# zrc0622/HIRL4UCAV

Hardware: AMD Instinct MI355X
Metric: env steps/sec (whole node) + HIRL update steps/sec at 4096 envs/GPU (higher is better)
Workload: dtype f32

## Files before the change

### hirl4ucav_amd/agents/engine.py

```python
import ctypes
import os

import numpy as np
import torch

from .. import _lib

H1, H2 = 256, 512
_vp, _i32, _f32 = ctypes.c_void_p, ctypes.c_int32, ctypes.c_float


class HxBatch(ctypes.Structure):
    _fields_ = [("rows", _vp), ("bc_rows", _vp), ("batch", _i32), ("noise", _vp)]


class HxSample(ctypes.Structure):
    _fields_ = [("total", _vp), ("cap", ctypes.c_int64), ("ring", _vp), ("expert_ring", _vp), ("expert_len", ctypes.c_int64),
                ("bc_table", _vp), ("bc_len", ctypes.c_int64), ("n_main", _i32), ("seed", ctypes.c_uint64), ("call", ctypes.c_uint32),
                ("sigma", _f32), ("idx", _vp), ("idx_bc", _vp), ("guard", ctypes.c_uint32)]


class HxFront(ctypes.Structure):
    _fields_ = [("flags", _vp), ("status", _vp), ("epoch", ctypes.c_uint32), ("with_c", ctypes.c_uint32)]

# ... 381 lines not shown
        B = self.batch
        if self.needs_reload:
            raise _lib.HxError("this engine failed after a front launch had been enqueued: load a snapshot before learn()")
        st = _lib.stream_ptr()
        pending, self._pending = self._pending, None
        pipe = getattr(before_exchange, "__self__", None) if before_exchange is not None else None
        if pending is not None and pipe is not None and (getattr(pipe, "_armed", None) is not None or getattr(pipe, "issued", False)):
            raise _lib.HxError("sample(defer=True) cannot be combined with an armed VectorStepPipeline: use sample(defer=False) when the "
                               "next env step may run beside learn()")
        if pending is not None and noise is not None:
            raise _lib.HxError("learn(noise=...) after sample(defer=True): the deferred draw produces the smoothing noise itself")
        noise = self._noise if noise is None else noise
        batch = HxBatch(self.rows.data_ptr(), self.bc_rows.data_ptr() if self.use_bc else None, B, noise.data_ptr())
        smp = ctypes.byref(pending[0]) if pending is not None else None
        nets, hyper = ctypes.byref(self.nets), ctypes.byref(self.hyper)
        if bc_weight_now is None:
            w_kind, w_given = 2, 0.0
        elif bc_weight_now == 100:
            w_kind, w_given = 1, 0.0
        else:
            w_kind, w_given = 0, float(bc_weight_now)
        actor_phase = self.actor_trainable
        self.critic_step += 1
        if actor_phase:
            self.actor_step += 1
            self.update_count += 1
        do_polyak = actor_phase and self.update_count % self.target_update_freq == 0
        if not self.staged:
            _lib.call("hx_hirl_learn_sampled", nets, ctypes.byref(batch), hyper, smp, self.critic_step, int(actor_phase), self.actor_step,
                      int(do_polyak), w_kind, w_given, float(bc_warm_up_weight), st)
        else:
            actor_fwd = (2 if w_kind == 1 else 1) if actor_phase else 0
            if smp is not None:
                grads = lambda: _lib.call("hx_hirl_critic_grads_sampled", nets, ctypes.byref(batch), hyper, smp, actor_fwd, st)
            else:
                grads = lambda: _lib.call("hx_hirl_critic_grads", nets, ctypes.byref(batch), hyper, actor_fwd, st)
            self._learn_staged(grads, batch, actor_phase, do_polyak, w_kind, w_given, bc_warm_up_weight, before_exchange)
        self.actor_trainable = not self.actor_trainable

    def _learn_staged(self, critic_grads, batch, actor_phase, do_polyak, w_kind, w_given, bc_warm_up_weight, before_exchange=None):
        B, st = self.batch, _lib.stream_ptr()
        nets, hyper = ctypes.byref(self.nets), ctypes.byref(self.hyper)
        gs = 1.0 / self.world
        own_critic = self.grad_critic.data_ptr()
        if self.xchg is not None:
            self.nets.grad_critic = self.xchg.write_buffer("critic").data_ptr()
        critic_grads()
        if before_exchange is not None:
            before_exchange()
        summed = self._allreduce(self.grad_critic, "critic")
        self.nets.grad_critic = summed.data_ptr()
        pk = 16 if do_polyak else 0
        _lib.call("hx_adam", nets, hyper, 0 | pk, self.critic_step, gs, 0, 0.0, 0.0, B, st)
        self.nets.grad_critic = own_critic
        if actor_phase:
            _lib.call("hx_hirl_actor_backward", nets, ctypes.byref(batch), hyper, int(w_kind == 1), 1, st)
            if self.world > 1 or self.sharded_sequence:
                if self.actor_msg is None:
                    self.actor_msg = torch.zeros(int(_lib.load().hx_actor_message_floats()), dtype=torch.float32, device=self.device)
                msg = self.xchg.write_buffer("actor") if self.xchg is not None else self.actor_msg
                _lib.call("hx_hirl_actor_wgrad_split", nets, hyper, B, msg.data_ptr(), st)
                summed = self._allreduce(msg, "actor")
                _lib.call("hx_adam_mixed", nets, hyper, int(do_polyak), self.actor_step, gs, w_kind, w_given, float(bc_warm_up_weight),
                          B * self.world, summed.data_ptr(), st)
            else:
                _lib.call("hx_hirl_actor_wgrad", nets, hyper, B, B, w_kind, w_given, float(bc_warm_up_weight), st)
                _lib.call("hx_adam", nets, hyper, 1 | pk, self.actor_step, gs, w_kind, w_given, float(bc_warm_up_weight), B, st)

    def step_learn(self, env, expert=None, bc_table=None, n_main=None, act_noise=None, act_sigma=0.0, act_seed=0, out=None, sample_seed=0,
                   smooth_sigma=0.2, bc_weight_now=0.0, bc_warm_up_weight=0.0):
        replay, n, B = env.replay, env.n, self.batch
        bf16 = self.update_dtype == "bf16"
        if replay is None or (self.act_dtype != "bf16" if bf16 else self.act_dtype not in ("f32", "f32x9")):
            raise _lib.HxError("step_learn: the front launch exists for the fp32 networks (acting format 'f32' or 'f32x9') and for the bf16 update path with "
                               "the bf16 acting format, with a replay ring attached to the env")
        if self._pending is not None:
            raise _lib.HxError("step_learn draws its own minibatch: a sample(defer=True) is still pending")
        if self._front is None:
            buf = torch.zeros(96, dtype=torch.int32, device=self.device)
            self._front = (buf[0:64], buf[64:65])
            second = torch.zeros(2 * B * 32 + 2 * B + 64, dtype=torch.float32, device=self.device)
            t2 = (second[:B * 32], second[B * 32:2 * B * 32], second[2 * B * 32:2 * B * 32 + B].view(torch.int32),
                  second[2 * B * 32 + B:2 * B * 32 + 2 * B].view(torch.int32), second[2 * B * 32 + 2 * B:2 * B * 32 + 2 * B + 4])
            self._front_tiles = [(self.rows, self.bc_rows, self._idx, self._idx_bc, self._noise), t2]
        flags, status = self._front
        cur, nxt = self._front_tiles
        n_main = B if n_main is None else int(n_main)
        if self.needs_reload:
            raise _lib.HxError("this engine failed after a front launch had been enqueued (host and device state may disagree): load a snapshot "
                               "(utils/checkpoint.load_run) before stepping it again")
        held = (self._front_epoch, self._front_c_epoch, self.critic_step, self.actor_step, self.update_count, self.sample_calls, self.act_calls, env.steps_issued)
        self._front_enqueued = False
        try:
            return self._step_learn(env, expert, bc_table, n_main, act_noise, act_sigma, act_seed, out, sample_seed, smooth_sigma, bc_weight_now,
                                    bc_warm_up_weight, bf16, flags, status, cur, nxt)
        except _lib.HxError:
            if self._front_enqueued:
                self.needs_reload = True
                raise
            (self._front_epoch, self._front_c_epoch, self.critic_step, self.actor_step, self.update_count, self.sample_calls, self.act_calls, env.steps_issued) = held
            self.front_reset()
            raise

    def _step_learn(self, env, expert, bc_table, n_main, act_noise, act_sigma, act_seed, out, sample_seed, smooth_sigma, bc_weight_now, bc_warm_up_weight,
                    bf16, flags, status, cur, nxt):
        replay, n, B = env.replay, env.n, self.batch
        self.sample_calls += 1

        def draw(tiles, call):
            return HxSample(replay.total.data_ptr(), replay.capacity, replay.ring.data_ptr(), expert.ring.data_ptr() if expert is not None else None,
                            len_of(expert), _lib.ptr(bc_table), bc_table.shape[0] if bc_table is not None else 0, n_main, int(sample_seed), call,
                            float(smooth_sigma), tiles[2].data_ptr(), tiles[3].data_ptr() if bc_table is not None else None, n)

        def tiles_of(t):
            return HxBatch(t[0].data_ptr(), t[1].data_ptr() if self.use_bc else None, B, t[4].data_ptr())

        want = (env, env.steps_issued, replay, expert, bc_table, n_main, int(sample_seed), float(smooth_sigma), self.sample_calls, n)
        if self._front_drawn != want:
            _lib.call("hx_sample_batch_guarded", replay.total.data_ptr(), replay.capacity, replay.ring.data_ptr(), expert.ring.data_ptr() if expert is not None else None,
                      len_of(expert), _lib.ptr(bc_table), bc_table.shape[0] if bc_table is not None else 0, B, n_main, 1, int(sample_seed), self.sample_calls,
                      float(smooth_sigma), cur[2].data_ptr(), cur[3].data_ptr() if bc_table is not None else None, cur[4].data_ptr(), cur[0].data_ptr(),
                      cur[1].data_ptr() if bc_table is not None else None, n, _lib.stream_ptr())
        if out is None:
            out = torch.empty((n, 4), dtype=torch.float32, device=self.device)
        mode = 0
        if act_noise is not None:
            mode = 1 if act_noise.numel() == 4 else 2
        elif act_sigma > 0:
            mode = 3
        self.act_calls += 1
        if self._front_epoch >= 200_000_000:
            flags.zero_()
            self._front_epoch = self._front_c_epoch = 0
        self._front_epoch += 1
        batch, nets, hyper, st = tiles_of(cur), ctypes.byref(self.nets), ctypes.byref(self.hyper), _lib.stream_ptr()
        if bc_weight_now is None:
            w_kind, w_given = 2, 0.0
        elif bc_weight_now == 100:
            w_kind, w_given = 1, 0.0
        else:
            w_kind, w_given = 0, float(bc_weight_now)
        actor_phase = self.actor_trainable
        self.critic_step += 1
        if actor_phase:
            self.actor_step += 1
            self.update_count += 1
        do_polyak = actor_phase and self.update_count % self.target_update_freq == 0
        with_c = int(self.front_c_for(n, actor_phase, w_kind, bf16))
        knob = os.environ.get("HX_FRONT_C")
        carries_c = knob == "1" or (bool(with_c) and knob != "0")
        if carries_c:
            self._front_c_epoch += 1
        front = HxFront(flags.data_ptr(), status.data_ptr(), self._front_epoch, self._front_c_epoch if carries_c else 0)
        _lib.call("hx_hirl_front", env.state.data_ptr(), n, env.pitch, env.obs.data_ptr(), out.data_ptr(), mode | self._mode_bits | (32 if (not bf16 and self._x9_for(n, front=True)) else 0),
                  _lib.ptr(act_noise), float(act_sigma), int(act_seed), int(env.env_id0), self.act_calls, env.reward.data_ptr(), env.done.data_ptr(),
                  env.success.data_ptr(), ctypes.byref(env._opts), nets, ctypes.byref(batch), hyper, int(actor_phase), w_kind, ctypes.byref(front), st)
        self._front_enqueued = True
        env.steps_issued += 1
        nxt_draw, nxt_tiles = draw(nxt, self.sample_calls + 1), tiles_of(nxt)
        if not self.staged:
            _lib.call("hx_hirl_learn_back", nets, ctypes.byref(batch), hyper, self.critic_step, int(actor_phase), self.actor_step, int(do_polyak), w_kind, w_given,
                      float(bc_warm_up_weight), ctypes.byref(nxt_draw), ctypes.byref(nxt_tiles), with_c, st)
        else:
            self._learn_staged(lambda: _lib.call("hx_hirl_critic_grads_back", nets, ctypes.byref(batch), hyper, ctypes.byref(nxt_draw), ctypes.byref(nxt_tiles), with_c, st),
                               batch, actor_phase, do_polyak, w_kind, w_given, bc_warm_up_weight)
        self._front_drawn = (env, env.steps_issued, replay, expert, bc_table, n_main, int(sample_seed), float(smooth_sigma), self.sample_calls + 1, n)
        self._front_tiles = [nxt, cur]
        self.rows, self.bc_rows, self._idx, self._idx_bc, self._noise = cur
        self.actor_trainable = not self.actor_trainable
        return out, env.obs, env.reward, env.done, env.success

    @staticmethod
    def front_waiting_workgroups(batch, with_c=False):
        tiles = (int(batch) + 15) // 16
        return 2 * tiles * 8 + (2 * ((int(batch) + 7) // 8) * 8 if with_c else 0)

    def front_c_for(self, n, actor_phase, w_kind, bf16):
        if self.front_c != "auto":
            return bool(self.front_c)
        if bf16 or not self._x9_for(n, front=True) or n < 8192 or n > 16384:
            return False
        acting = (n + 63) // 64
        jobs = (3 + 2) + (1 + (0 if not self.use_bc else (2 if w_kind == 1 else 1)))
        tiles = (self.batch + 15) // 16
        need = jobs * tiles * 8 * 6.0 + 2 * ((self.batch + 7) // 8) * 8 * 7.6
        return (256 - acting) * 37.0 >= need

    def front_reset(self):
        if self._front is not None:
            self._front[0].zero_()
            self._front[1].zero_()
        self._front_epoch = self._front_c_epoch = 0
        self._front_drawn = None

    def front_status(self):
        return 0 if self._front is None else int(self._front[1].item())

    def front_check(self):
        code = self.front_status()
        if code != 0:
            which = [w for bit, w in ((1, "launch B for the target actor's rows (launch A)"), (2, "launch C for the rows of launches A / B")) if code & bit]
            raise _lib.HxError(f"front launch: an in-launch wait timed out (status word {code}: " + "; ".join(which) + ") - the minibatches read since are "
                               "suspect; the reference-order loop (train_all --loop reference) has no in-launch waits")

    def bc_train_actor(self):
        batch = HxBatch(self.rows.data_ptr(), self.bc_rows.data_ptr(), self.batch, self._noise.data_ptr())
        self.actor_step += 1
        _lib.call("hx_bc_train_actor", ctypes.byref(self.nets), ctypes.byref(batch), ctypes.byref(self.hyper), self.actor_step, _lib.stream_ptr())

    def losses_host(self):
        v = self.losses.tolist()
        return v[0], v[1], v[2], v[3], v[4], v[5]
```

### hirl4ucav_amd/csrc/hx_fwdbwd.hip

```cpp
#include "hx_bwd_body.h"

using namespace hxnn;
using namespace hxu;

namespace {

template <int NT, bool RELU, bool SAMPLE, bool BF16 = false>
__global__ __launch_bounds__(kWide) void fwd_l2_kernel(FwdArgsC A, typename std::conditional<SAMPLE, SampleDev, NoSample>::type SA) {
    __shared__ FwdLds<NT, SAMPLE, BF16> SL;
    fwd_l2_body<NT, RELU, SAMPLE, BF16, 0>(A, SA, (int)blockIdx.x, (int)blockIdx.y, SL, FrontSync{});
}

template <int GRP, bool RELU, bool BF16 = false>
__global__ __launch_bounds__(kWide) void bwd_l2_kernel(BwdArgsC AC) {
    __shared__ BwdLds<GRP, BF16> SL;
    bwd_l2_body<GRP, RELU, BF16, 0>(AC, (int)blockIdx.x, (int)blockIdx.y, SL, FrontSync{});
}


int fwd_row_tiles(const FwdArgs& a) {
    int n = 0;
    for (int j = 0; j < a.njobs; ++j) n += (a.job[j].rows + RT - 1) / RT;
    return n;
}
int bwd_blocks(const BwdArgs& a, int rows_per_wg) {
    return ((a.job[0].rows + rows_per_wg - 1) / rows_per_wg) * kColWgB;
}
template <int GRP>
void launch_bwd_t(const BwdArgs& G, hipStream_t st) {
    BwdArgsC C{};
    for (int j = 0; j < G.njobs; ++j) C.job[j] = pack_bwd(G.job[j], G);
    C.images = G.images;
    static const int rowmap = getenv("HX_XCD_ROWMAP") ? atoi(getenv("HX_XCD_ROWMAP")) : 3;
    C.rowmap = (rowmap >> 1) & 1;
    const dim3 grid(bwd_blocks(G, (GRP <= 2 || GRP >= 4) ? RT / 2 : RT) , G.njobs);
    if constexpr (GRP <= 2) {
        static const int dbg_off = getenv("HX_DBG_BF16_OFF") ? atoi(getenv("HX_DBG_BF16_OFF")) : 0;
        if (G.images && !(dbg_off & 2)) {
            if (G.slope == 0.0f) hipLaunchKernelGGL((bwd_l2_kernel<GRP, true, true>), grid, dim3(kWide), 0, st, C);
            else hipLaunchKernelGGL((bwd_l2_kernel<GRP, false, true>), grid, dim3(kWide), 0, st, C);
            return;
        }
    }
    if (G.slope == 0.0f) hipLaunchKernelGGL((bwd_l2_kernel<GRP, true>), grid, dim3(kWide), 0, st, C);
    else hipLaunchKernelGGL((bwd_l2_kernel<GRP, false>), grid, dim3(kWide), 0, st, C);
}

}

namespace hxu {

static int g_force_fwd_nt = 0, g_force_skip = 0, g_force_count = 0;
void set_fwd_nt(int nt, int skip, int count) { g_force_fwd_nt = nt; g_force_skip = skip; g_force_count = count; }

void launch_fwd(const FwdArgs& F, hipStream_t st) {
    static const bool env64 = getenv("HX_FWD_NT64") && atoi(getenv("HX_FWD_NT64")) != 0;
    bool force64 = env64;
    if (g_force_fwd_nt == kNT) {
        if (g_force_skip > 0) --g_force_skip;
        else if (g_force_count > 0) { --g_force_count; force64 = true; }
    }
    FwdArgsC C{};
    for (int j = 0; j < F.njobs; ++j) {
        C.job[j] = pack_fwd(F.job[j]);
        C.job[j].slope = F.slope;
    }
    C.slope = F.slope; C.zero_nf = F.zero_nf; C.zero_f = F.zero_f; C.zero_i = F.zero_i; C.images = F.images;
    static const int rowmap = getenv("HX_XCD_ROWMAP") ? atoi(getenv("HX_XCD_ROWMAP")) : 3;
    C.rowmap = rowmap & 1;
    const int tiles = fwd_row_tiles(F), per_job = tiles / F.njobs;
    const bool relu = F.slope == 0.0f;
    static const int dbg_off = getenv("HX_DBG_BF16_OFF") ? atoi(getenv("HX_DBG_BF16_OFF")) : 0;
    const bool bf16 = F.images != nullptr && !(dbg_off & 1);
#define HX_FWD_T(NT_, RELU_, BF16_) hipLaunchKernelGGL((fwd_l2_kernel<NT_, RELU_, false, BF16_>), grid, dim3(kWide), 0, st, C, NoSample{})
#define HX_FWD(NT_) do { const dim3 grid(per_job * (H2 / NT_), F.njobs); \
        if (bf16) { if (relu) HX_FWD_T(NT_, true, true); else HX_FWD_T(NT_, false, true); } \
        else { if (relu) HX_FWD_T(NT_, true, false); else HX_FWD_T(NT_, false, false); } } while (0)
    if (F.sample) {
        const dim3 grid(per_job * (H2 / kNT), F.njobs);
        if (bf16) {
            if (relu) hipLaunchKernelGGL((fwd_l2_kernel<kNT, true, true, true>), grid, dim3(kWide), 0, st, C, *F.sample);
            else hipLaunchKernelGGL((fwd_l2_kernel<kNT, false, true, true>), grid, dim3(kWide), 0, st, C, *F.sample);
        } else {
            if (relu) hipLaunchKernelGGL((fwd_l2_kernel<kNT, true, true>), grid, dim3(kWide), 0, st, C, *F.sample);
            else hipLaunchKernelGGL((fwd_l2_kernel<kNT, false, true>), grid, dim3(kWide), 0, st, C, *F.sample);
        }
        return;
    }
    if (tiles >= 128) HX_FWD(256);
    else if (tiles * (H2 / 32) <= 256 && !force64) HX_FWD(32);
    else HX_FWD(kNT);
#undef HX_FWD_T
#undef HX_FWD
}

void launch_bwd(int grp, const BwdArgs& G, hipStream_t st) {
    switch (grp) {
        case 0: launch_bwd_t<0>(G, st); break;
        case 1: launch_bwd_t<1>(G, st); break;
        case 2: launch_bwd_t<2>(G, st); break;
        case 4: launch_bwd_t<4>(G, st); break;
        case 5: launch_bwd_t<5>(G, st); break;
        default: launch_bwd_t<3>(G, st); break;
    }
}

}

HX_DEFINE_DEBUG_COLLECTORS(fwdbwd, 0, 32)

extern "C" int hx_debug_set_fwd_nt(int32_t nt, int32_t skip, int32_t count) {
    HX_REQUIRE((nt == 0 || nt == 64) && skip >= 0 && count >= 0, "hx_debug_set_fwd_nt: nt 0 or 64, skip and count >= 0");
    hxu::set_fwd_nt(nt, skip, count);
    return 0;
}
```

### hirl4ucav_amd/csrc/hx_hirl.hip

```cpp
#include <cmath>

#include "hx_update.h"

using namespace hxnn;
using namespace hxu;

extern "C" {

int hx_actor_param_count(void) { return kActor.size(); }
int hx_critic_param_count(void) { return 2 * kQ.padded(); }
int64_t hx_hirl_workspace_floats(int32_t batch) { return (int64_t)S_COUNT * kSlotFloats * batch + 64; }
int64_t hx_actor_message_floats(void) { return 2 * (int64_t)kActor.padded() + 64; }
int64_t hx_bf16_images_elems(void) { return (int64_t)IM_COUNT * (int64_t)kImgElems; }

int hx_pack_update_images(const HxNets* N, void* stream) {
    HX_REQUIRE(N && N->w2_bf16_all && (reinterpret_cast<uintptr_t>(N->w2_bf16_all) & 15u) == 0, "hx_pack_update_images: w2_bf16_all must be a 16-byte aligned buffer");
    HX_REQUIRE(N->actor && N->critic && N->target_actor && N->target_critic, "hx_pack_update_images: null network");
    hipStream_t st = (hipStream_t)stream;
    uint16_t* im = N->w2_bf16_all;
    launch_pack_bf16(N->actor + kActor.W2(), im + IM_ACTOR * kImgElems, false, st);
    launch_pack_bf16(N->actor + kActor.W2(), im + IM_ACTOR_T * kImgElems, true, st);
    launch_pack_bf16(N->target_actor + kActor.W2(), im + IM_TA * kImgElems, false, st);
    if (N->bc_actor) launch_pack_bf16(N->bc_actor + kActor.W2(), im + IM_BC * kImgElems, false, st);
    for (int h = 0; h < 2; ++h) {
        launch_pack_bf16(N->critic + h * kQ.padded() + kQ.W2(), im + (IM_C1 + h) * kImgElems, false, st);
        launch_pack_bf16(N->critic + h * kQ.padded() + kQ.W2(), im + (IM_C1_T + h) * kImgElems, true, st);
        launch_pack_bf16(N->target_critic + h * kQ.padded() + kQ.W2(), im + (IM_TC1 + h) * kImgElems, false, st);
    }
    HX_CHECK_LAUNCH("hx_pack_update_images");
    return 0;
}

static void make_slots(const HxNets* N, int B, Slot* s) {
    for (int i = 0; i < S_COUNT; ++i) s[i] = carve_slot(N->ws + (size_t)i * kSlotFloats * B, B);
}

static WgAdam make_adam(const HxNets* N, const HxHyper* Hy, float lr, int step, bool finish_actor) {
    const double b1 = 0.9, b2 = 0.999;
    const double bc1 = 1.0 - pow(b1, step), bc2 = 1.0 - pow(b2, step);
    WgAdam a{};
    a.b1 = (float)b1; a.b2 = (float)b2; a.eps = 1e-8f;
    a.step_size = (float)(lr / bc1);
    a.bc2_sqrt = (float)sqrt(bc2);
    a.tau = Hy->tau;
    a.finish_actor = finish_actor ? 1 : 0;
    a.use_bc = Hy->use_bc;
    a.losses = N->losses;
    a.wstate = N->wstate;
    return a;
}

static void make_launch_a(const HxNets* N, const HxBatch* Bt, const HxHyper* Hy, int32_t actor_fwd, FwdArgs& F) {
    const Mlp mA{13, 4, Hy->no_layernorm ? 1 : 0}, mQ{17, 1, Hy->no_layernorm ? 1 : 0};
    const int B = Bt->batch;
    Slot s[S_COUNT];
    make_slots(N, B, s);
    const RowSrc src{Bt->rows, nullptr, nullptr, 0, 32};
    F = FwdArgs{};
    F.njobs = 3; F.slope = Hy->slope;
    F.zero_f = N->losses; F.zero_nf = 1;
    F.job[0] = FwdJob{N->target_actor, mA, src, 17, 0, Head{}, nullptr, 0.f, s[S_TA], B, 0, IM_TA};
    F.job[1] = FwdJob{N->critic, mQ, src, 0, 0, Head{}, nullptr, 0.f, s[S_C1], B, 1, IM_C1};
    F.job[2] = FwdJob{N->critic + mQ.padded(), mQ, src, 0, 0, Head{}, nullptr, 0.f, s[S_C2], B, 1, IM_C2};
    if (actor_fwd) {
        F.zero_nf = 5; F.zero_i = N->soft_count;
        F.job[3] = FwdJob{N->actor, mA, src, 0, 0, Head{}, nullptr, 0.f, s[S_API], B, 1, IM_ACTOR};
        F.njobs = 4;
    }
    F.images = N->w2_bf16_all;
}
static void make_launch_b(const HxNets* N, const HxBatch* Bt, const HxHyper* Hy, int32_t actor_fwd, FwdArgs& F) {
    const Mlp mA{13, 4, Hy->no_layernorm ? 1 : 0}, mQ{17, 1, Hy->no_layernorm ? 1 : 0};
    const int B = Bt->batch;
    Slot s[S_COUNT];
    make_slots(N, B, s);
    const RowSrc src{Bt->rows, nullptr, nullptr, 0, 32};
    const float* tc1 = N->target_critic;
    const float* tc2 = N->target_critic + mQ.padded();
    F = FwdArgs{};
    F.njobs = 2; F.slope = Hy->slope;
    const Head prev{N->target_actor, mA, s[S_TA]};
    F.job[0] = FwdJob{tc1, mQ, src, 17, 1, prev, Bt->noise, Hy->noise_clamp, s[S_TC1], B, 0, IM_TC1};
    F.job[1] = FwdJob{tc2, mQ, src, 17, 1, prev, Bt->noise, Hy->noise_clamp, s[S_TC2], B, 0, IM_TC2};
    if (actor_fwd && Hy->use_bc) {
        const RowSrc bcsrc{Bt->bc_rows ? Bt->bc_rows : Bt->rows, nullptr, nullptr, 0, 32};
        int n = 2;
        F.job[n++] = FwdJob{N->actor, mA, bcsrc, 0, 0, Head{}, nullptr, 0.f, s[S_ABC], B, 1, IM_ACTOR};
        if (actor_fwd == 2) F.job[n++] = FwdJob{N->bc_actor, mA, src, 0, 0, Head{}, nullptr, 0.f, s[S_BCS], B, 0, IM_BC};
        F.njobs = n;
    }
    F.images = N->w2_bf16_all;
}
static void make_launch_c(const HxNets* N, const HxBatch* Bt, const HxHyper* Hy, BwdArgs& G) {
    const Mlp mQ{17, 1, Hy->no_layernorm ? 1 : 0};
    const int B = Bt->batch;
    Slot s[S_COUNT];
    make_slots(N, B, s);
    const RowSrc src{Bt->rows, nullptr, nullptr, 0, 32};
    const float* tc1 = N->target_critic;
    const float* tc2 = N->target_critic + mQ.padded();
    G = BwdArgs{};
    G.njobs = 2; G.slope = Hy->slope; G.inv_batch = 1.0f / B; G.losses = N->losses; G.soft_count = N->soft_count;
    for (int h = 0; h < 2; ++h) {
        BwdJob& J = G.job[h];
        J = BwdJob{};
        J.net = N->critic + h * mQ.padded(); J.m = mQ; J.ws = s[S_C1 + h]; J.rows = B; J.mode = BM_CRITIC_TD;
        J.t1 = Head{tc1, mQ, s[S_TC1]}; J.t2 = Head{tc2, mQ, s[S_TC2]}; J.src = src; J.gamma = Hy->gamma;
        J.img_t = IM_C1_T + h;
    }
    G.images = N->w2_bf16_all;
}
static bool front_has_c(bool asked) {
    static const int force = getenv("HX_FRONT_C") ? atoi(getenv("HX_FRONT_C")) : -1;
    return force < 0 ? asked : force != 0;
}
static int critic_back(const HxNets* N, const HxBatch* Bt, const HxHyper* Hy, void* stream, int adam_step, bool polyak, const SampleDev* predraw = nullptr, bool skip_c = false) {
    hipStream_t st = (hipStream_t)stream;
    const Mlp mQ{17, 1, Hy->no_layernorm ? 1 : 0};
    const int B = Bt->batch;
    Slot s[S_COUNT];
    make_slots(N, B, s);
    if (!skip_c) {
        BwdArgs G;
        make_launch_c(N, Bt, Hy, G);
        launch_bwd(0, G, st);
    }
    {
        WgArgs W{};
        W.njobs = 2; W.slope = Hy->slope; W.w_kind = 0; W.w_given = 0.f; W.inv_batch = 1.0f / B;
        W.soft_count = N->soft_count; W.wstate = N->wstate;
        for (int h = 0; h < 2; ++h) {
            WgJob& J = W.job[h];
            J = WgJob{};
            J.net = N->critic + h * mQ.padded(); J.grad = N->grad_critic + h * mQ.padded(); J.m = mQ;
            J.ws[0] = s[S_C1 + h]; J.rows[0] = B; J.nslots = 1; J.wmode[0] = 0;
            if (adam_step > 0) {
                J.p = N->critic + h * mQ.padded();
                J.mom = N->m_critic + h * mQ.padded(); J.var = N->v_critic + h * mQ.padded();
                J.target = polyak ? N->target_critic + h * mQ.padded() : nullptr;
                if (uint16_t* im = N->w2_bf16_all) {
                    J.w2b = im + (IM_C1 + h) * kImgElems; J.w2tb = im + (IM_C1_T + h) * kImgElems; J.tgt_w2b = im + (IM_TC1 + h) * kImgElems;
                }
            }
        }
        W.bf16 = N->w2_bf16_all != nullptr;
        W.predraw = predraw; W.predraw_batch = B;
        if (adam_step > 0) {
            W.ad = make_adam(N, Hy, Hy->lr_critic, adam_step, false);
            launch_wg(W, true, st);
        } else {
            launch_wg(W, false, st);
        }
    }
    HX_CHECK_LAUNCH("hx_hirl_critic_grads");
    return 0;
}
static int critic_grads_impl(const HxNets* N, const HxBatch* Bt, const HxHyper* Hy, int32_t actor_fwd, void* stream, int adam_step, bool polyak,
                             const HxSample* S = nullptr) {
    HX_REQUIRE(N && Bt && Hy && Bt->batch > 0 && Bt->batch % 16 == 0, "hx_hirl_critic_grads: batch must be a positive multiple of 16");
    hipStream_t st = (hipStream_t)stream;
    const int B = Bt->batch;
    SampleDev SD{};
    bool fused = false;
    if (S) {
        HX_REQUIRE(Bt->noise, "hx_hirl_*_sampled: the draw needs the output word noise[4]");
        if (int rc = prepare_draw(S, B, const_cast<float*>(Bt->rows), const_cast<float*>(Bt->bc_rows), const_cast<float*>(Bt->noise), stream, &SD, &fused)) return rc;
    }
    FwdArgs F;
    make_launch_a(N, Bt, Hy, actor_fwd, F);
    F.sample = fused ? &SD : nullptr;
    launch_fwd(F, st);
    make_launch_b(N, Bt, Hy, actor_fwd, F);
    launch_fwd(F, st);
    return critic_back(N, Bt, Hy, stream, adam_step, polyak);
}
int hx_hirl_critic_grads(const HxNets* N, const HxBatch* Bt, const HxHyper* Hy, int32_t actor_fwd, void* stream) {
    return critic_grads_impl(N, Bt, Hy, actor_fwd, stream, 0, false);
}
int hx_hirl_critic_grads_sampled(const HxNets* N, const HxBatch* Bt, const HxHyper* Hy, const HxSample* S, int32_t actor_fwd, void* stream) {
    HX_REQUIRE(S, "hx_hirl_critic_grads_sampled: null sample description");
    return critic_grads_impl(N, Bt, Hy, actor_fwd, stream, 0, false, S);
}

int hx_hirl_actor_backward(const HxNets* N, const HxBatch* Bt, const HxHyper* Hy, int32_t estimate_soft, int32_t fwd_done, void* stream) {
    HX_REQUIRE(N && Bt && Hy && Bt->batch > 0 && Bt->batch % 16 == 0, "hx_hirl_actor_backward: batch must be a positive multiple of 16");
    hipStream_t st = (hipStream_t)stream;
    const Mlp mA{13, 4, Hy->no_layernorm ? 1 : 0}, mQ{17, 1, Hy->no_layernorm ? 1 : 0};
    (void)mA; (void)mQ;
    const int B = Bt->batch;
    Slot s[S_COUNT];
    make_slots(N, B, s);
    const RowSrc src{Bt->rows, nullptr, nullptr, 0, 32};
    const RowSrc bcsrc{Bt->bc_rows ? Bt->bc_rows : Bt->rows, nullptr, nullptr, 0, 32};
    const bool bc = Hy->use_bc != 0, soft = bc && estimate_soft;
    if (!fwd_done) {
        FwdArgs F{};
        F.slope = Hy->slope;
        F.zero_f = N->losses + 1; F.zero_nf = 4; F.zero_i = N->soft_count;
        int n = 0;
        F.job[n++] = FwdJob{N->actor, mA, src, 0, 0, Head{}, nullptr, 0.f, s[S_API], B, 1, IM_ACTOR};
        if (bc) F.job[n++] = FwdJob{N->actor, mA, bcsrc, 0, 0, Head{}, nullptr, 0.f, s[S_ABC], B, 1, IM_ACTOR};
        if (soft) F.job[n++] = FwdJob{N->bc_actor, mA, src, 0, 0, Head{}, nullptr, 0.f, s[S_BCS], B, 0, IM_BC};
        F.njobs = n;
        F.images = N->w2_bf16_all;
        launch_fwd(F, st);
    }
    {
        FwdArgs F{};
        F.slope = Hy->slope;
        int n = 0;
        F.job[n++] = FwdJob{N->critic, mQ, src, 0, 1, Head{N->actor, mA, s[S_API]}, nullptr, 0.f, s[S_CPI], B, 1, IM_C1};
        if (soft) F.job[n++] = FwdJob{N->critic, mQ, src, 0, 1, Head{N->bc_actor, mA, s[S_BCS]}, nullptr, 0.f, s[S_CSOFT], B, 0, IM_C1};
        F.njobs = n;
        F.images = N->w2_bf16_all;
        launch_fwd(F, st);
    }
    {
        BwdArgs G{};
        G.njobs = 1; G.slope = Hy->slope; G.inv_batch = 1.0f / B; G.losses = N->losses; G.soft_count = N->soft_count;
        BwdJob& J = G.job[0];
        J = BwdJob{};
        J.net = N->critic; J.m = mQ; J.ws = s[S_CPI]; J.rows = B; J.mode = BM_CRITIC_PI;
        if (soft) J.soft = Head{N->critic, mQ, s[S_CSOFT]};
        J.img_t = IM_C1_T;
        G.images = N->w2_bf16_all;
        launch_bwd(1, G, st);
    }
    {
        BwdArgs G{};
        G.slope = Hy->slope; G.inv_batch = 1.0f / B; G.losses = N->losses; G.soft_count = N->soft_count;
        int n = 0;
        {
            BwdJob& J = G.job[n++];
            J = BwdJob{};
            J.net = N->actor; J.m = mA; J.ws = s[S_API]; J.rows = B; J.mode = BM_ACTOR_PI;
            J.crit = Head{N->critic, mQ, s[S_CPI]};
            J.img_t = IM_ACTOR_T;
        }
        if (bc) {
            BwdJob& J = G.job[n++];
            J = BwdJob{};
            J.net = N->actor; J.m = mA; J.ws = s[S_ABC]; J.rows = B; J.mode = BM_ACTOR_BC;
            J.src = bcsrc; J.lambda = Hy->loss_lambda;
            J.img_t = IM_ACTOR_T;
        }
        G.njobs = n;
        G.images = N->w2_bf16_all;
        launch_bwd(2, G, st);
    }
    HX_CHECK_LAUNCH("hx_hirl_actor_backward");
    return 0;
}

static int actor_wgrad_impl(const HxNets* N, const HxHyper* Hy, int32_t batch, int32_t count_batch, int32_t w_kind, float w_given,
                            float warm, void* stream, int adam_step, bool polyak) {
    HX_REQUIRE(N && Hy && batch > 0 && count_batch > 0, "hx_hirl_actor_wgrad: bad arguments");
    const Mlp mA{13, 4, Hy->no_layernorm ? 1 : 0}, mQ{17, 1, Hy->no_layernorm ? 1 : 0};
    (void)mA; (void)mQ;
    Slot s[S_COUNT];
    make_slots(N, batch, s);
    const bool bc = Hy->use_bc != 0;
    WgArgs W{};
    W.njobs = 1; W.slope = Hy->slope; W.w_kind = bc ? w_kind : 0; W.w_given = bc ? w_given : 0.0f; W.warm = warm;
    W.inv_batch = 1.0f / count_batch; W.soft_count = N->soft_count; W.wstate = N->wstate;
    WgJob& J = W.job[0];
    J = WgJob{};
    J.net = N->actor; J.grad = N->grad_actor; J.m = mA;
    J.ws[0] = s[S_API]; J.rows[0] = batch; J.wmode[0] = 1;
    J.nslots = 1;
    if (bc) { J.ws[1] = s[S_ABC]; J.rows[1] = batch; J.wmode[1] = 2; J.nslots = 2; }
    W.bf16 = N->w2_bf16_all != nullptr;
    if (adam_step > 0) {
        J.p = N->actor; J.mom = N->m_actor; J.var = N->v_actor;
        J.target = polyak ? N->target_actor : nullptr;
        J.w2b = N->actor_w2_bf16;
        J.w2f = N->actor_w2_f32i;
        if (N->actor_w2_x9) {
            HX_REQUIRE(!N->actor_w2_bf16 && !N->w2_bf16_all, "hx_hirl_learn: actor_w2_x9 excludes the plain bf16 images (one acting format at a time)");
            J.w2b = N->actor_w2_x9; J.w2b_x9 = 1;
        }
        if (uint16_t* im = N->w2_bf16_all) {
            HX_REQUIRE(!N->actor_w2_bf16 || N->actor_w2_bf16 == im + IM_ACTOR * kImgElems, "hx_hirl_learn: with w2_bf16_all set, actor_w2_bf16 must be NULL or its first image");
            J.w2b = im + IM_ACTOR * kImgElems; J.w2tb = im + IM_ACTOR_T * kImgElems; J.tgt_w2b = im + IM_TA * kImgElems;
        }
        W.ad = make_adam(N, Hy, Hy->lr_actor, adam_step, true);
        launch_wg(W, true, (hipStream_t)stream);
    } else {
        launch_wg(W, false, (hipStream_t)stream);
    }
    HX_CHECK_LAUNCH("hx_hirl_actor_wgrad");
    return 0;
}
int hx_hirl_actor_wgrad(const HxNets* N, const HxHyper* Hy, int32_t batch, int32_t count_batch, int32_t w_kind, float w_given,
                        float warm, void* stream) {
    return actor_wgrad_impl(N, Hy, batch, count_batch, w_kind, w_given, warm, stream, 0, false);
}

int hx_hirl_actor_wgrad_split(const HxNets* N, const HxHyper* Hy, int32_t batch, float* msg, void* stream) {
    HX_REQUIRE(N && Hy && batch > 0 && msg && (reinterpret_cast<uintptr_t>(msg) & 15u) == 0, "hx_hirl_actor_wgrad_split: bad arguments");
    const Mlp mA{13, 4, Hy->no_layernorm ? 1 : 0}, mQ{17, 1, Hy->no_layernorm ? 1 : 0};
    (void)mA; (void)mQ;
    Slot s[S_COUNT];
    make_slots(N, batch, s);
    const bool bc = Hy->use_bc != 0;
    WgArgs W{};
    W.njobs = bc ? 2 : 1; W.slope = Hy->slope; W.w_kind = 0; W.w_given = 0.0f; W.inv_batch = 1.0f / batch;
    W.soft_count = N->soft_count; W.wstate = N->wstate;
    for (int j = 0; j < W.njobs; ++j) {
        WgJob& J = W.job[j];
        J = WgJob{};
        J.net = N->actor; J.grad = msg + j * mA.padded(); J.m = mA;
        J.ws[0] = s[j == 0 ? S_API : S_ABC]; J.rows[0] = batch; J.wmode[0] = 0; J.nslots = 1;
    }
    W.bf16 = N->w2_bf16_all != nullptr;
    W.soft_count = bc ? N->soft_count : nullptr;
    W.count_out = msg + 2 * mA.padded();
    launch_wg(W, false, (hipStream_t)stream);
    HX_CHECK_LAUNCH("hx_hirl_actor_wgrad_split");
    return 0;
}

int hx_hirl_learn(const HxNets* N, const HxBatch* Bt, const HxHyper* Hy, int32_t critic_step, int32_t actor_phase,
                  int32_t actor_step, int32_t do_polyak, int32_t w_kind, float w_given, float warm, void* stream) {
    return hx_hirl_learn_sampled(N, Bt, Hy, nullptr, critic_step, actor_phase, actor_step, do_polyak, w_kind, w_given, warm, stream);
}
int hx_hirl_learn_sampled(const HxNets* N, const HxBatch* Bt, const HxHyper* Hy, const HxSample* S, int32_t critic_step, int32_t actor_phase,
                          int32_t actor_step, int32_t do_polyak, int32_t w_kind, float w_given, float warm, void* stream) {
    HX_REQUIRE(critic_step >= 1 && (!actor_phase || actor_step >= 1), "hx_hirl_learn: Adam steps are 1-based");
    int rc = critic_grads_impl(N, Bt, Hy, actor_phase ? (w_kind == 1 ? 2 : 1) : 0, stream, critic_step, do_polyak != 0, S);
    if (rc || !actor_phase) return rc;
    if ((rc = hx_hirl_actor_backward(N, Bt, Hy, w_kind == 1, 1, stream))) return rc;
    return actor_wgrad_impl(N, Hy, Bt->batch, Bt->batch, w_kind, w_given, warm, stream, actor_step, do_polyak != 0);
}

int hx_hirl_front(float* state, int64_t n, int64_t stride, float* obs_io, float* actions, int32_t noise_mode, const float* noise,
                  float sigma, uint64_t seed, uint32_t row0, uint32_t call, float* reward, uint8_t* done, int8_t* success, const HxStepOpts* opts,
                  const HxNets* N, const HxBatch* Bt, const HxHyper* Hy, int32_t actor_phase, int32_t w_kind, const HxFront* front, void* stream) {
    HX_REQUIRE(N && Bt && Hy && front && opts && Bt->batch > 0 && Bt->batch % 16 == 0 && Bt->batch <= kFusedBatchMax && Bt->rows && Bt->noise,
               "hx_hirl_front: the minibatch tiles (a positive multiple of 16 rows, at most 256) and noise[4] must be there");
    HX_REQUIRE(front->flags && front->status && front->epoch >= 1, "hx_hirl_front: flags, status and a 1-based epoch are required");
    const bool bf16 = N->w2_bf16_all != nullptr;
    HX_REQUIRE(bf16 ? N->actor_w2_bf16 != nullptr : (!N->actor_w2_bf16 && (N->actor_w2_f32i || N->actor_w2_x9)),
               "hx_hirl_front: fp32 networks with HxNets.actor_w2_f32i / actor_w2_x9, or the bf16 update path (w2_bf16_all) with actor_w2_bf16");
    const int actor_fwd = actor_phase ? (w_kind == 1 ? 2 : 1) : 0;
    FwdArgs FA, FB;
    make_launch_a(N, Bt, Hy, actor_fwd, FA);
    make_launch_b(N, Bt, Hy, actor_fwd, FB);
    const bool x9 = !bf16 && (noise_mode & 32) != 0;
    HX_REQUIRE(bf16 || (x9 ? N->actor_w2_x9 != nullptr : N->actor_w2_f32i != nullptr), "hx_hirl_front: the image of the chosen acting format is missing from HxNets");
    noise_mode &= ~32;
    BwdArgs GC;
    const bool with_c = front_has_c(front->with_c != 0);
    HX_REQUIRE(!with_c || front->with_c != 0, "hx_hirl_front: HX_FRONT_C=1 needs a caller that counts its launches with launch C (HxFront.with_c = 1, 2, ...)");
    if (with_c) make_launch_c(N, Bt, Hy, GC);
    return launch_front(N->actor, (x9 || bf16) ? nullptr : N->actor_w2_f32i, x9 ? N->actor_w2_x9 : nullptr, bf16 ? N->actor_w2_bf16 : nullptr, state, n, stride, obs_io, actions, noise_mode, noise, sigma, seed,
                        row0, call, Hy->slope, reward, done, success, *opts, FA, FB, with_c ? &GC : nullptr, *front, (hipStream_t)stream);
}
static int make_predraw(const HxNets* N, const HxBatch* Bt, const HxSample* next, const HxBatch* next_tiles, void* stream, SampleDev* SD) {
    HX_REQUIRE(next_tiles && next_tiles->batch == Bt->batch && next_tiles->rows && next_tiles->noise && next_tiles->rows != Bt->rows && next_tiles->noise != Bt->noise,
               "hx_hirl_learn_back: the next minibatch needs tiles of its own (this call still reads the current ones)");
    (void)N;
    bool fused = false;
    if (int rc = prepare_draw(next, Bt->batch, const_cast<float*>(next_tiles->rows), const_cast<float*>(next_tiles->bc_rows), const_cast<float*>(next_tiles->noise),
                              stream, SD, &fused, false)) return rc;
    HX_REQUIRE(fused, "hx_hirl_learn_back: the predraw covers minibatches of at most 256 rows");
    return 0;
}
int hx_hirl_critic_grads_back(const HxNets* N, const HxBatch* Bt, const HxHyper* Hy, const HxSample* next, const HxBatch* next_tiles, int32_t c_in_front,
                              void* stream) {
    HX_REQUIRE(N && Bt && Hy && Bt->batch > 0 && Bt->batch % 16 == 0, "hx_hirl_critic_grads_back: batch must be a positive multiple of 16");
    SampleDev SD{};
    if (next) if (int rc = make_predraw(N, Bt, next, next_tiles, stream, &SD)) return rc;
    return critic_back(N, Bt, Hy, stream, 0, false, next ? &SD : nullptr, front_has_c(c_in_front != 0));
}
int hx_hirl_learn_back(const HxNets* N, const HxBatch* Bt, const HxHyper* Hy, int32_t critic_step, int32_t actor_phase, int32_t actor_step, int32_t do_polyak,
                       int32_t w_kind, float w_given, float warm, const HxSample* next, const HxBatch* next_tiles, int32_t c_in_front, void* stream) {
    HX_REQUIRE(N && Bt && Hy && Bt->batch > 0 && Bt->batch % 16 == 0, "hx_hirl_learn_back: batch must be a positive multiple of 16");
    HX_REQUIRE(critic_step >= 1 && (!actor_phase || actor_step >= 1), "hx_hirl_learn_back: Adam steps are 1-based");
    SampleDev SD{};
    if (next) if (int rc = make_predraw(N, Bt, next, next_tiles, stream, &SD)) return rc;
    int rc = critic_back(N, Bt, Hy, stream, critic_step, do_polyak != 0, next ? &SD : nullptr, front_has_c(c_in_front != 0));
    if (rc || !actor_phase) return rc;
    if ((rc = hx_hirl_actor_backward(N, Bt, Hy, w_kind == 1, 1, stream))) return rc;
    return actor_wgrad_impl(N, Hy, Bt->batch, Bt->batch, w_kind, w_given, warm, stream, actor_step, do_polyak != 0);
}

int hx_bc_train_actor(const HxNets* N, const HxBatch* Bt, const HxHyper* Hy, int32_t step, void* stream) {
    HX_REQUIRE(N && Bt && Hy && Bt->bc_rows && Bt->batch > 0 && Bt->batch % 16 == 0 && step >= 1, "hx_bc_train_actor: bad arguments");
    hipStream_t st = (hipStream_t)stream;
    const Mlp mA{13, 4, Hy->no_layernorm ? 1 : 0}, mQ{17, 1, Hy->no_layernorm ? 1 : 0};
    (void)mA; (void)mQ;
    const int B = Bt->batch;
    Slot s[S_COUNT];
    make_slots(N, B, s);
    const RowSrc bcsrc{Bt->bc_rows, nullptr, nullptr, 0, 32};
    {
        FwdArgs F{};
        F.njobs = 1; F.slope = Hy->slope;
        F.zero_f = N->losses + 1; F.zero_nf = 4;
        F.job[0] = FwdJob{N->actor, mA, bcsrc, 0, 0, Head{}, nullptr, 0.f, s[S_ABC], B, 1, IM_ACTOR};
        F.images = N->w2_bf16_all;
        launch_fwd(F, st);
    }
    {
        BwdArgs G{};
        G.njobs = 1; G.slope = Hy->slope; G.inv_batch = 1.0f / B; G.losses = N->losses; G.soft_count = N->soft_count;
        BwdJob& J = G.job[0];
        J = BwdJob{};
        J.net = N->actor; J.m = mA; J.ws = s[S_ABC]; J.rows = B; J.mode = BM_ACTOR_BC; J.src = bcsrc; J.lambda = 1.0f;
        J.img_t = IM_ACTOR_T;
        G.images = N->w2_bf16_all;
        launch_bwd(2, G, st);
    }
    {
        WgArgs W{};
        W.njobs = 1; W.slope = Hy->slope; W.w_kind = 0; W.w_given = 0.f; W.inv_batch = 1.0f / B;
        W.soft_count = N->soft_count; W.wstate = N->wstate;
        WgJob& J = W.job[0];
        J = WgJob{};
        J.net = N->actor; J.grad = N->grad_actor; J.m = mA; J.ws[0] = s[S_ABC]; J.rows[0] = B; J.nslots = 1; J.wmode[0] = 0;
        W.bf16 = N->w2_bf16_all != nullptr;
        launch_wg(W, false, st);
    }
    HX_CHECK_LAUNCH("hx_bc_train_actor");
    return hx_adam(N, Hy, 2, step, 1.0f, 0, 0.0f, 0.0f, B, stream);
}

}
```

### hirl4ucav_amd/csrc/hx_update.h

```cpp
#pragma once
#include <cstdlib>
#include <type_traits>

#include "hx_common.h"
#include "hx_nn.h"

#ifdef HX_STAMPS
static __device__ float hx_dbg[80];
#define STAMP_DECL unsigned long long TS_[16]; int tsn_ = 0
#define STAMP() TS_[tsn_++] = __builtin_amdgcn_s_memrealtime()
#define STAMP_FLUSH(base, cond) do { if (cond) { for (int i_ = 1; i_ < tsn_; ++i_) hx_dbg[(base) + i_] = (float)(TS_[i_] - TS_[i_ - 1]); hx_dbg[(base)] = (float)tsn_; } } while (0)
constexpr int kSpanCap = 8192;
static __device__ unsigned long long hx_span[kSpanCap][2];
static __device__ unsigned hx_span_tag[kSpanCap];
static __device__ unsigned hx_span_n;
#define SPAN_LOG(tag) do { if (threadIdx.x == 0) { const unsigned long long e_ = __builtin_amdgcn_s_memrealtime(); const unsigned i_ = atomicAdd(&hx_span_n, 1u); \
    if (i_ < (unsigned)kSpanCap) { hx_span[i_][0] = TS_[0]; hx_span[i_][1] = e_; hx_span_tag[i_] = (unsigned)(tag) | (blockIdx.x << 8) | (blockIdx.y << 24); } } } while (0)
#define HX_DEFINE_DEBUG_COLLECTORS(name, lo, hi) \
    namespace hx { \
    int dbg_stamps_##name(float* host80) { \
        float tmp[80]; \
        if (hipMemcpyFromSymbol(tmp, HIP_SYMBOL(hx_dbg), sizeof(tmp)) != hipSuccess) return -2; \
        for (int i = (lo); i < (hi); ++i) host80[i] = tmp[i]; \
        return 0; \
// ... 428 lines not shown
#pragma clang fp contract(off)
__device__ __forceinline__ void sac_policy_dout(float da, float a, float se, float mask, float ab, float& d_mean, float& d_logstd) {
    const float t = 1.0f - a * a;
    const float dHdx = (-2.0f * a * t) / (t + 1e-6f);
    const float dLdx = da * t - ab * dHdx;
    d_mean = dLdx;
    d_logstd = (dLdx * se - ab) * mask;
}
#pragma clang fp contract(fast)

struct BwdJob {
    const float* net;
    Mlp m;
    Slot ws;
    int rows;
    int mode;
    Head t1, t2;
    RowSrc src;
    float gamma;
    Head soft;
    Head crit;
    float lambda;
    const float* bonus;
    const float* bonus_scale;
    int loss_slot;
    int img_t;
};
struct BwdArgs {
    BwdJob job[2];
    int njobs;
    float slope;
    float inv_batch;
    float* losses;
    int* soft_count;
    const uint16_t* images;
};

struct WgJob {
    const float* net;
    float* grad;
    Mlp m;
    Slot ws[2];
    int rows[2];
    int nslots;
    int wmode[2];
    float* p; float* mom; float* var;
    float* target;
    uint16_t* w2b;
    float* w2f;
    uint16_t* w2tb;
    uint16_t* tgt_w2b;
    int w2b_x9;
};
struct WgAdam {
    float b1, b2, eps, step_size, bc2_sqrt, tau;
    int finish_actor, use_bc;
    float* losses;
    float* wstate;
    float* alpha_state;
    float target_entropy, alpha_step_size;
};
struct WgArgs {
    WgJob job[2];
    int njobs;
    float slope;
    WgAdam ad;
    int w_kind;
    float w_given, warm, inv_batch;
    const int* soft_count;
    const float* wstate;
    int bf16;
    float* count_out;
    const SampleDev* predraw;
    int predraw_batch;
};

#pragma clang fp contract(off)
__device__ __forceinline__ void adam_update(float& p, float& m, float& v, float g, float b1, float b2, float eps, float step_size, float bc2_sqrt) {
    m = __builtin_fmaf(g, 1.0f - b1, m * b1);
    v = __builtin_fmaf(g * g, 1.0f - b2, v * b2);
    const float denom = __builtin_amdgcn_sqrtf(v) * __builtin_amdgcn_rcpf(bc2_sqrt) + eps;
    p = p - step_size * (m * __builtin_amdgcn_rcpf(denom));
}
__device__ __forceinline__ float polyak_update(float target, float p, float tau) { return target * (1.0f - tau) + p * tau; }
#pragma clang fp contract(fast)
__device__ __forceinline__ float effective_w(int kind, float given, float warm, float inv_batch, const int* count, const float* wstate) {
    float w = given;
    if (kind == 1) w = (float)(*count) * inv_batch + warm;
    if (kind == 2) w = *wstate;
    return w > 1.0f ? 1.0f : w;
}

struct AdamArgs {
    float* p; const float* g; float* m; float* v;
    int n;
    float b1, b2, eps, step_size, bc2_sqrt, gscale;
    int finish_actor;
    int w_kind; float w_given, warm, inv_batch;
    const int* soft_count; float* wstate; float* losses; int use_bc;
    float* alpha_state;
    float target_entropy, alpha_step_size;
    float* target;
    float tau;
    uint16_t* w2b;
    float* w2f;
    int w2b_x9;
    int w2_lo;
    int nseg;
    int seg_lo[2];
    uint16_t* seg_w2b[2];
    uint16_t* seg_w2tb[2];
    uint16_t* seg_tgt_w2b[2];
    const float* g2;
    const float* countf;
    const uint32_t* guard;
};

constexpr size_t kSlotFloats = XP + H1 + 2 + H1 + H2 + 2 + OW + H2 + H1 + OW + 2 * kColWgB;

enum { S_TA = 0, S_C1, S_C2, S_TC1, S_TC2, S_API, S_ABC, S_BCS, S_CPI, S_CSOFT, S_COUNT };

const Mlp kActor{13, 4, 0};
const Mlp kQ{17, 1, 0};
const Mlp kPolicy{13, 8, 1};
const Mlp kQs{17, 1, 1};

__device__ __forceinline__ float pick8(const float (&o)[8], int i) {
    return i == 0 ? o[0] : i == 1 ? o[1] : i == 2 ? o[2] : i == 3 ? o[3] : i == 4 ? o[4] : i == 5 ? o[5] : i == 6 ? o[6] : o[7];
}

inline int prepare_draw(const HxSample* S, int B, float* rows, float* bc_rows, float* noise, void* stream, SampleDev* SD, bool* fused, bool launch_now = true) {
    HX_REQUIRE(S->total && S->cap > 0 && S->ring && S->idx && rows && S->n_main >= 0 && S->n_main <= B,
               "hx_*_sampled: the draw needs total, cap, ring, idx and the output tile rows");
    HX_REQUIRE(S->n_main == B || S->expert_ring, "hx_*_sampled: expert rows requested without an expert ring");
    HX_REQUIRE(!S->bc_table == !S->idx_bc && (!S->bc_table || bc_rows), "hx_*_sampled: bc_table, idx_bc and bc_rows go together");
    *fused = B <= kFusedBatchMax;
    HX_REQUIRE(!S->guard || *fused, "hx_*_sampled: HxSample.guard is honoured by the fused draw only (batch <= 256)");
    HX_REQUIRE(!S->guard || 2 * (int64_t)S->guard <= S->cap, "hx_*_sampled: a guard of more than half the ring leaves too little to draw from (cap >= 2 n)");
    if (*fused) {
        *SD = SampleDev{(const unsigned long long*)S->total, S->ring, S->expert_ring ? S->expert_ring : S->ring, S->bc_table, rows,
                        S->bc_table ? bc_rows : nullptr, noise, S->idx, S->idx_bc, (long long)S->cap, (uint32_t)S->expert_len, (uint32_t)S->bc_len,
                        S->n_main, S->call, S->seed, S->sigma, S->guard};
        return 0;
    }
    if (!launch_now) return 0;
    return hx_sample_batch(S->total, S->cap, S->ring, S->expert_ring, S->expert_len, S->bc_table, S->bc_len, B, S->n_main, 1, S->seed, S->call,
                           S->sigma, S->idx, S->idx_bc, noise, rows, S->bc_table ? bc_rows : nullptr, stream);
}


void launch_fwd(const FwdArgs& F, hipStream_t st);
void set_fwd_nt(int nt, int skip, int count);
void launch_bwd(int grp, const BwdArgs& G, hipStream_t st);
int launch_front(const float* actor, const float* w2f, const uint16_t* w2x, const uint16_t* w2b, float* state, int64_t n, int64_t stride, float* obs_io, float* actions, int32_t noise_mode,
                 const float* noise, float sigma, uint64_t seed, uint32_t row0, uint32_t call, float slope, float* reward, uint8_t* done, int8_t* success,
                 const HxStepOpts& o, const FwdArgs& FA, const FwdArgs& FB, const BwdArgs* GC, const HxFront& front, hipStream_t st);
void launch_wg(const WgArgs& W, bool adam, hipStream_t st);
void launch_adam(const AdamArgs& A, hipStream_t st);
void launch_polyak(float* target, const float* source, int n, float tau, float* target2, const float* source2, int n2, hipStream_t st,
                   const uint32_t* guard = nullptr);
void launch_pack_bf16(const float* w2, uint16_t* image, bool transposed, hipStream_t st);

}
```

Before: 79.59 million.

## Move BC actor forward from front launch B into actor backward launch H

In the non-staged actor phase with behaviour cloning enabled, the BC-rows actor forward job is removed from the front's launch B. It is instead co-launched with the first actor backward layer-2 kernel in one grid, where some blocks run the backward and the rest run the forward, sharing LDS through a union. This shortens the front's forward launch and fills the backward launch with independent work. The risk is a larger LDS footprint and uneven block mix in the combined kernel, plus the BC forward output now being ready later than before.

After: 79.67 million (median of 6 runs). No clear change (+0.1%).

```diff
diff --git a/hirl4ucav_amd/agents/engine.py b/hirl4ucav_amd/agents/engine.py
--- a/hirl4ucav_amd/agents/engine.py
+++ b/hirl4ucav_amd/agents/engine.py
@@ -557,7 +557,8 @@
         if carries_c:
             self._front_c_epoch += 1
         front = HxFront(flags.data_ptr(), status.data_ptr(), self._front_epoch, self._front_c_epoch if carries_c else 0)
-        _lib.call("hx_hirl_front", env.state.data_ptr(), n, env.pitch, env.obs.data_ptr(), out.data_ptr(), mode | self._mode_bits | (32 if (not bf16 and self._x9_for(n, front=True)) else 0),
+        sbc_in_h = not self.staged and actor_phase and self.use_bc
+        _lib.call("hx_hirl_front", env.state.data_ptr(), n, env.pitch, env.obs.data_ptr(), out.data_ptr(), mode | self._mode_bits | (32 if (not bf16 and self._x9_for(n, front=True)) else 0) | (64 if sbc_in_h else 0),
                   _lib.ptr(act_noise), float(act_sigma), int(act_seed), int(env.env_id0), self.act_calls, env.reward.data_ptr(), env.done.data_ptr(),
                   env.success.data_ptr(), ctypes.byref(env._opts), nets, ctypes.byref(batch), hyper, int(actor_phase), w_kind, ctypes.byref(front), st)
         self._front_enqueued = True
@@ -565,7 +566,7 @@
         nxt_draw, nxt_tiles = draw(nxt, self.sample_calls + 1), tiles_of(nxt)
         if not self.staged:
             _lib.call("hx_hirl_learn_back", nets, ctypes.byref(batch), hyper, self.critic_step, int(actor_phase), self.actor_step, int(do_polyak), w_kind, w_given,
-                      float(bc_warm_up_weight), ctypes.byref(nxt_draw), ctypes.byref(nxt_tiles), with_c, st)
+                      float(bc_warm_up_weight), ctypes.byref(nxt_draw), ctypes.byref(nxt_tiles), with_c | (2 if sbc_in_h else 0), st)
         else:
             self._learn_staged(lambda: _lib.call("hx_hirl_critic_grads_back", nets, ctypes.byref(batch), hyper, ctypes.byref(nxt_draw), ctypes.byref(nxt_tiles), with_c, st),
                                batch, actor_phase, do_polyak, w_kind, w_given, bc_warm_up_weight)
diff --git a/hirl4ucav_amd/csrc/hx_fwdbwd.hip b/hirl4ucav_amd/csrc/hx_fwdbwd.hip
--- a/hirl4ucav_amd/csrc/hx_fwdbwd.hip
+++ b/hirl4ucav_amd/csrc/hx_fwdbwd.hip
@@ -15,6 +15,20 @@
 __global__ __launch_bounds__(kWide) void bwd_l2_kernel(BwdArgsC AC) {
     __shared__ BwdLds<GRP, BF16> SL;
     bwd_l2_body<GRP, RELU, BF16, 0>(AC, (int)blockIdx.x, (int)blockIdx.y, SL, FrontSync{});
+}
+
+template <bool RELU, bool BF16>
+__global__ __launch_bounds__(kWide) void bwd1_fwd_kernel(BwdArgsC AC, int nb, FwdArgsC F) {
+    __shared__ union {
+        BwdLds<1, BF16> b;
+        FwdLds<kNT, false, BF16> f;
+    } u;
+    const int b = (int)blockIdx.x;
+    if (b < nb) {
+        bwd_l2_body<1, RELU, BF16, 0>(AC, b, 0, u.b, FrontSync{});
+        return;
+    }
+    fwd_l2_body<kNT, RELU, false, BF16, 0>(F, NoSample{}, b - nb, 0, u.f, FrontSync{});
 }
 
 
@@ -94,6 +108,30 @@
 #undef HX_FWD
 }
 
+int launch_bwd1_fwd(const BwdArgs& G, const FwdArgs& F, hipStream_t st) {
+    HX_REQUIRE(G.njobs == 1 && F.njobs == 1 && !F.sample && F.zero_nf == 0 && !F.zero_i && F.job[0].rows == G.job[0].rows && !G.images == !F.images,
+               "launch_bwd1_fwd: one backward job of launch H and one forward job on the same minibatch, the same update path");
+    BwdArgsC C{};
+    C.job[0] = pack_bwd(G.job[0], G);
+    C.images = G.images;
+    static const int rowmap = getenv("HX_XCD_ROWMAP") ? atoi(getenv("HX_XCD_ROWMAP")) : 3;
+    C.rowmap = (rowmap >> 1) & 1;
+    FwdArgsC A{};
+    A.job[0] = pack_fwd(F.job[0]);
+    A.job[0].slope = F.slope;
+    A.slope = F.slope; A.images = F.images; A.rowmap = rowmap & 1;
+    const int nb = bwd_blocks(G, RT / 2), nf = ((F.job[0].rows + RT - 1) / RT) * (H2 / kNT);
+    const dim3 grid((unsigned)(nb + nf));
+    if (G.images) {
+        if (G.slope == 0.0f) hipLaunchKernelGGL((bwd1_fwd_kernel<true, true>), grid, dim3(kWide), 0, st, C, nb, A);
+        else hipLaunchKernelGGL((bwd1_fwd_kernel<false, true>), grid, dim3(kWide), 0, st, C, nb, A);
+    } else {
+        if (G.slope == 0.0f) hipLaunchKernelGGL((bwd1_fwd_kernel<true, false>), grid, dim3(kWide), 0, st, C, nb, A);
+        else hipLaunchKernelGGL((bwd1_fwd_kernel<false, false>), grid, dim3(kWide), 0, st, C, nb, A);
+    }
+    return 0;
+}
+
 void launch_bwd(int grp, const BwdArgs& G, hipStream_t st) {
     switch (grp) {
         case 0: launch_bwd_t<0>(G, st); break;
diff --git a/hirl4ucav_amd/csrc/hx_hirl.hip b/hirl4ucav_amd/csrc/hx_hirl.hip
--- a/hirl4ucav_amd/csrc/hx_hirl.hip
+++ b/hirl4ucav_amd/csrc/hx_hirl.hip
@@ -69,7 +69,7 @@
     }
     F.images = N->w2_bf16_all;
 }
-static void make_launch_b(const HxNets* N, const HxBatch* Bt, const HxHyper* Hy, int32_t actor_fwd, FwdArgs& F) {
+static void make_launch_b(const HxNets* N, const HxBatch* Bt, const HxHyper* Hy, int32_t actor_fwd, FwdArgs& F, bool sbc_in_h = false) {
     const Mlp mA{13, 4, Hy->no_layernorm ? 1 : 0}, mQ{17, 1, Hy->no_layernorm ? 1 : 0};
     const int B = Bt->batch;
     Slot s[S_COUNT];
@@ -85,7 +85,7 @@
     if (actor_fwd && Hy->use_bc) {
         const RowSrc bcsrc{Bt->bc_rows ? Bt->bc_rows : Bt->rows, nullptr, nullptr, 0, 32};
         int n = 2;
-        F.job[n++] = FwdJob{N->actor, mA, bcsrc, 0, 0, Head{}, nullptr, 0.f, s[S_ABC], B, 1, IM_ACTOR};
+        if (!sbc_in_h) F.job[n++] = FwdJob{N->actor, mA, bcsrc, 0, 0, Head{}, nullptr, 0.f, s[S_ABC], B, 1, IM_ACTOR};
         if (actor_fwd == 2) F.job[n++] = FwdJob{N->bc_actor, mA, src, 0, 0, Head{}, nullptr, 0.f, s[S_BCS], B, 0, IM_BC};
         F.njobs = n;
     }
@@ -182,7 +182,7 @@
     return critic_grads_impl(N, Bt, Hy, actor_fwd, stream, 0, false, S);
 }
 
-int hx_hirl_actor_backward(const HxNets* N, const HxBatch* Bt, const HxHyper* Hy, int32_t estimate_soft, int32_t fwd_done, void* stream) {
+static int actor_backward_impl(const HxNets* N, const HxBatch* Bt, const HxHyper* Hy, int32_t estimate_soft, int32_t fwd_done, void* stream, bool sbc_in_h) {
     HX_REQUIRE(N && Bt && Hy && Bt->batch > 0 && Bt->batch % 16 == 0, "hx_hirl_actor_backward: batch must be a positive multiple of 16");
     hipStream_t st = (hipStream_t)stream;
     const Mlp mA{13, 4, Hy->no_layernorm ? 1 : 0}, mQ{17, 1, Hy->no_layernorm ? 1 : 0};
@@ -224,7 +224,14 @@
         if (soft) J.soft = Head{N->critic, mQ, s[S_CSOFT]};
         J.img_t = IM_C1_T;
         G.images = N->w2_bf16_all;
-        launch_bwd(1, G, st);
+        if (sbc_in_h && bc) {
+            FwdArgs F{};
+            F.slope = Hy->slope; F.njobs = 1; F.images = N->w2_bf16_all;
+            F.job[0] = FwdJob{N->actor, mA, bcsrc, 0, 0, Head{}, nullptr, 0.f, s[S_ABC], B, 1, IM_ACTOR};
+            if (int rc = launch_bwd1_fwd(G, F, st)) return rc;
+        } else {
+            launch_bwd(1, G, st);
+        }
     }
     {
         BwdArgs G{};
@@ -250,6 +257,9 @@
     }
     HX_CHECK_LAUNCH("hx_hirl_actor_backward");
     return 0;
+}
+int hx_hirl_actor_backward(const HxNets* N, const HxBatch* Bt, const HxHyper* Hy, int32_t estimate_soft, int32_t fwd_done, void* stream) {
+    return actor_backward_impl(N, Bt, Hy, estimate_soft, fwd_done, stream, false);
 }
 
 static int actor_wgrad_impl(const HxNets* N, const HxHyper* Hy, int32_t batch, int32_t count_batch, int32_t w_kind, float w_given,
@@ -345,7 +355,8 @@
     const int actor_fwd = actor_phase ? (w_kind == 1 ? 2 : 1) : 0;
     FwdArgs FA, FB;
     make_launch_a(N, Bt, Hy, actor_fwd, FA);
-    make_launch_b(N, Bt, Hy, actor_fwd, FB);
+    make_launch_b(N, Bt, Hy, actor_fwd, FB, (noise_mode & 64) != 0);
+    noise_mode &= ~64;
     const bool x9 = !bf16 && (noise_mode & 32) != 0;
     HX_REQUIRE(bf16 || (x9 ? N->actor_w2_x9 != nullptr : N->actor_w2_f32i != nullptr), "hx_hirl_front: the image of the chosen acting format is missing from HxNets");
     noise_mode &= ~32;
@@ -371,7 +382,7 @@
     HX_REQUIRE(N && Bt && Hy && Bt->batch > 0 && Bt->batch % 16 == 0, "hx_hirl_critic_grads_back: batch must be a positive multiple of 16");
     SampleDev SD{};
     if (next) if (int rc = make_predraw(N, Bt, next, next_tiles, stream, &SD)) return rc;
-    return critic_back(N, Bt, Hy, stream, 0, false, next ? &SD : nullptr, front_has_c(c_in_front != 0));
+    return critic_back(N, Bt, Hy, stream, 0, false, next ? &SD : nullptr, front_has_c((c_in_front & 1) != 0));
 }
 int hx_hirl_learn_back(const HxNets* N, const HxBatch* Bt, const HxHyper* Hy, int32_t critic_step, int32_t actor_phase, int32_t actor_step, int32_t do_polyak,
                        int32_t w_kind, float w_given, float warm, const HxSample* next, const HxBatch* next_tiles, int32_t c_in_front, void* stream) {
@@ -379,9 +390,9 @@
     HX_REQUIRE(critic_step >= 1 && (!actor_phase || actor_step >= 1), "hx_hirl_learn_back: Adam steps are 1-based");
     SampleDev SD{};
     if (next) if (int rc = make_predraw(N, Bt, next, next_tiles, stream, &SD)) return rc;
-    int rc = critic_back(N, Bt, Hy, stream, critic_step, do_polyak != 0, next ? &SD : nullptr, front_has_c(c_in_front != 0));
+    int rc = critic_back(N, Bt, Hy, stream, critic_step, do_polyak != 0, next ? &SD : nullptr, front_has_c((c_in_front & 1) != 0));
     if (rc || !actor_phase) return rc;
-    if ((rc = hx_hirl_actor_backward(N, Bt, Hy, w_kind == 1, 1, stream))) return rc;
+    if ((rc = actor_backward_impl(N, Bt, Hy, w_kind == 1, 1, stream, (c_in_front & 2) != 0))) return rc;
     return actor_wgrad_impl(N, Hy, Bt->batch, Bt->batch, w_kind, w_given, warm, stream, actor_step, do_polyak != 0);
 }
 
diff --git a/hirl4ucav_amd/csrc/hx_update.h b/hirl4ucav_amd/csrc/hx_update.h
--- a/hirl4ucav_amd/csrc/hx_update.h
+++ b/hirl4ucav_amd/csrc/hx_update.h
@@ -604,6 +604,7 @@
 void launch_fwd(const FwdArgs& F, hipStream_t st);
 void set_fwd_nt(int nt, int skip, int count);
 void launch_bwd(int grp, const BwdArgs& G, hipStream_t st);
+int launch_bwd1_fwd(const BwdArgs& G, const FwdArgs& F, hipStream_t st);
 int launch_front(const float* actor, const float* w2f, const uint16_t* w2x, const uint16_t* w2b, float* state, int64_t n, int64_t stride, float* obs_io, float* actions, int32_t noise_mode,
                  const float* noise, float sigma, uint64_t seed, uint32_t row0, uint32_t call, float slope, float* reward, uint8_t* done, int8_t* success,
                  const HxStepOpts& o, const FwdArgs& FA, const FwdArgs& FB, const BwdArgs* GC, const HxFront& front, hipStream_t st);
```
